# kamenbliznashki/chexpert

Hardware: AMD Instinct MI355X
Metric: images/sec fwd+bwd DenseNet121 320x320 bf16 (per-GPU rate in config.images_per_sec_per_gpu) (higher is better)
Workload: dtype bf16; 1 GPU; densenet121 bf16 1xMI355X 320x320 bs=256 per GPU, U-Ones labels (BASELINE configs[1]); 14 classes; random-init weights, synthetic uint8 X-rays; per_gpu_batch=256, global_batch=256, parallelism=dp1, rccl_ranks=1, capture_failed=0, launch=hipGraph replay

## Files before the change

### chexpert_amd/csrc/conv3x3_strip.hip

```cpp
#include <cstdlib>
#include "common.h"

namespace {

constexpr int XP_FWD = 272;
constexpr int XP_WG = 320;
constexpr int NCHX = 7;

struct StripGeo {
  int B, H, W, P, R, Q;
  int spi;
  int steps_per_wg;
};

__device__ __forceinline__ int wrapq(int v, int q) { return v >= q ? v - q : v; }

__global__ __launch_bounds__(192, 2) void conv3x3_strip_fwd_kernel(const bf16* __restrict__ x, int ldx,
                                                                 const float* __restrict__ sc, const float* __restrict__ sh,
                                                                 const bf16* __restrict__ wpk, bf16* __restrict__ y, int ldy,
                                                                 float* stat_sum, float* stat_sq, int stat_replicas, int stat_rstride,
                                                                 int stat_det, const StripGeo g) {
  extern __shared__ __attribute__((aligned(16))) char smem[];
  float* coef = reinterpret_cast<float*>(smem);
  float* lstat = coef + 256;
  float* scratch = lstat + 64;
  char* ring = reinterpret_cast<char*>(scratch + 3 * 1024);
  const int tid = threadIdx.x, lane = tid & 63, wave = tid >> 6;
  const int P = g.P, R = g.R, Q = g.Q, W = g.W, H = g.H;

  bf16x8 wr[3][8];
#pragma unroll
  for (int dx = 0; dx < 3; ++dx)
#pragma unroll
    for (int ks = 0; ks < 8; ++ks)
      wr[dx][ks] = *reinterpret_cast<const bf16x8*>(wpk + ((size_t)((wave * 3 + dx) * 32 + (lane & 31)) * 128 + ks * 16 + (lane >> 5) * 8));
  for (int i = tid; i < (Q + 2) * (XP_FWD / 16); i += 192) reinterpret_cast<uint4*>(ring)[i] = make_uint4(0, 0, 0, 0);
  for (int i = tid; i < 128; i += 192) { coef[i] = sc[i]; coef[128 + i] = sh[i]; }
  if (tid < 64) lstat[tid] = 0.f;
  __syncthreads();

  const int total_steps = g.B * g.spi;
  const int u0 = blockIdx.x * g.steps_per_wg;
  const int u1 = min(total_steps, u0 + g.steps_per_wg);
  const int chunks_per_row = W * 16;

  uint4 pre[NCHX];
  bool pv[NCHX];
  int base_row = 0;
  int crow[NCHX], cpx[NCHX], cc8[NCHX];
#pragma unroll
  for (int i = 0; i < NCHX; ++i) {
    const int cid = tid + 192 * i;
    crow[i] = cid / chunks_per_row;
    const int rem = cid - crow[i] * chunks_per_row;
    cpx[i] = rem >> 4;
    cc8[i] = rem & 15;
  }
  auto issue_rows = [&](int b, int y0, int n) {
#pragma unroll
    for (int i = 0; i < NCHX; ++i) {
      const int yy = y0 + crow[i];
      pv[i] = crow[i] < n && yy >= 0 && yy < H;
      const int yc_ = min(max(yy, 0), H - 1);
      pre[i] = *reinterpret_cast<const uint4*>(x + ((size_t)(b * H + yc_) * W + cpx[i]) * ldx + cc8[i] * 8);
    }
  };
  auto write_rows = [&](int y0, int n) {
#pragma unroll
    for (int i = 0; i < NCHX; ++i) {
      if (crow[i] < n) {
        int slot = (y0 + crow[i] - base_row) % (R + 2);
        if (slot < 0) slot += R + 2;
        U128 o, v;
        v.u = pre[i];
#pragma unroll
        for (int j = 0; j < 8; ++j)
          o.e[j] = f2bf(fmaxf(fmaf(bf2f(v.e[j]), coef[cc8[i] * 8 + j], coef[128 + cc8[i] * 8 + j]), 0.f));
        { const unsigned keep = pv[i] ? 0xffffffffu : 0u; o.u.x &= keep; o.u.y &= keep; o.u.z &= keep; o.u.w &= keep; }
        const int pos = slot * P + cpx[i] + 1;
        *reinterpret_cast<uint4*>(ring + pos * XP_FWD + cc8[i] * 16) = o.u;
        if (pos < 2) *reinterpret_cast<uint4*>(ring + (Q + pos) * XP_FWD + cc8[i] * 16) = o.u;
      }
    }
  };

  float s1[8], s2[8];
#pragma unroll
  for (int j = 0; j < 8; ++j) s1[j] = s2[j] = 0.f;
  const int nsub = (R * P + 31) / 32;
  bool have_window = false;
  int prev_b = -1, prev_yc = 0;

  for (int u = u0; u < u1; ++u) {
    const int b = u / g.spi, yc = (u - b * g.spi) * R;
    const bool cont = have_window && b == prev_b && yc == prev_yc + R;
    if (!cont) {
      __syncthreads();
      base_row = yc - 1;
      issue_rows(b, yc - 1, 1);
      write_rows(yc - 1, 1);
      issue_rows(b, yc, 1);
      write_rows(yc, 1);
      issue_rows(b, yc + 1, R);
    }
    write_rows(yc + 1, R);
    __syncthreads();
    const bool next_cont = (u + 1 < u1) && ((u + 1) / g.spi == b);
    if (next_cont) issue_rows(b, yc + R + 1, R);
    int slot0 = (yc - 1 - base_row) % (R + 2);
    if (slot0 < 0) slot0 += R + 2;
    const int ws = slot0 * P;

    for (int s = 0; s < nsub; ++s) {
      f32x16 acc;
#pragma unroll
      for (int r = 0; r < 16; ++r) acc[r] = 0.f;
      {
        const int pix = min(s * 32 + (lane & 31), R * P - 1);
        const char* ap = ring + wrapq(wrapq(ws + pix + wave * P, Q), Q) * XP_FWD + (lane >> 5) * 16;
#pragma unroll
        for (int dx = 0; dx < 3; ++dx)
#pragma unroll
          for (int ks = 0; ks < 8; ++ks) {
            const bf16x8 a = *reinterpret_cast<const bf16x8*>(ap + dx * XP_FWD + ks * 32);
            acc = __builtin_amdgcn_mfma_f32_32x32x16_bf16(a, wr[dx][ks], acc, 0, 0, 0);
          }
      }
      float* my = scratch + wave * 1024;
#pragma unroll
      for (int r = 0; r < 16; ++r) my[((r & 3) + 8 * (r >> 2) + 4 * (lane >> 5)) * 32 + (lane & 31)] = acc[r];
      __syncthreads();
      if (tid < 128) {
        const int pr = tid >> 2, c = tid & 3;
        const int m = s * 32 + pr;
        const int oy = m / P, ox = m - oy * P;
        const int yy = yc + oy;
        if (m < R * P && ox < W && yy < H) {
          float v[8];
#pragma unroll
          for (int j = 0; j < 8; ++j) v[j] = 0.f;
#pragma unroll
          for (int w3 = 0; w3 < 3; ++w3) {
            const float4 v0 = *reinterpret_cast<const float4*>(scratch + w3 * 1024 + pr * 32 + c * 8);
            const float4 v1 = *reinterpret_cast<const float4*>(scratch + w3 * 1024 + pr * 32 + c * 8 + 4);
            v[0] += v0.x; v[1] += v0.y; v[2] += v0.z; v[3] += v0.w;
            v[4] += v1.x; v[5] += v1.y; v[6] += v1.z; v[7] += v1.w;
          }
          U128 o;
#pragma unroll
          for (int j = 0; j < 8; ++j) {
            o.e[j] = f2bf(v[j]);
            const float rv = bf2f(o.e[j]);
            s1[j] += rv;
            s2[j] += rv * rv;
          }
          *reinterpret_cast<uint4*>(y + ((size_t)(b * H + yy) * W + ox) * ldy + c * 8) = o.u;
        }
      }
      __syncthreads();
    }
    have_window = true;
    prev_b = b;
    prev_yc = yc;
  }

  if (stat_sum) {
#pragma unroll
    for (int j = 0; j < 8; ++j) {
#pragma unroll
      for (int d = 4; d < 64; d <<= 1) {
        s1[j] += __shfl_xor(s1[j], d);
        s2[j] += __shfl_xor(s2[j], d);
      }
    }
    wg_stat_begin<3>(scratch, 32, tid, 192);
    if (lane < 4 && wave < 2) {
#pragma unroll
      for (int j = 0; j < 8; ++j) wg_stat_put(scratch, 32, wave, lane * 8 + j, s1[j], s2[j]);
    }
    wg_stat_end<3>(scratch, 32, tid, 192, stat_sum, stat_sq, stat_det, (int)blockIdx.x, stat_replicas, stat_rstride, 0, 32);
  }
}

constexpr int GP = 80;
constexpr int NCHD = 2;

__global__ __launch_bounds__(192, 2) void conv3x3_strip_dgrad_kernel(
    const bf16* __restrict__ gsl, int ldg, const bf16* __restrict__ g2, int ldg2, const float* __restrict__ ga,
    const float* __restrict__ gb, const float* __restrict__ gc, const bf16* __restrict__ wpk, const bf16* __restrict__ ex, int ldex,
    const float* __restrict__ e_sc, const float* __restrict__ e_sh, const float* __restrict__ e_mu, const float* __restrict__ e_r,
    const float* __restrict__ e_scale, bf16* __restrict__ y, int ldy, float* S1, float* S2, int stat_replicas, int stat_rstride,
    int stat_det, const StripGeo g) {
  extern __shared__ __attribute__((aligned(16))) char smem[];
  float* coef = reinterpret_cast<float*>(smem);
  float* lstat = coef + 128;
  float* econst = lstat + 256;
  float* scratch = econst + 640;
  char* ring = reinterpret_cast<char*>(scratch + 3 * 4096);
  const int tid = threadIdx.x, lane = tid & 63, wave = tid >> 6;
  const int P = g.P, R = g.R, Q = g.Q, W = g.W, H = g.H;

  bf16x8 wr[3][2][4];
#pragma unroll
  for (int dx = 0; dx < 3; ++dx)
#pragma unroll
    for (int ks = 0; ks < 2; ++ks)
#pragma unroll
      for (int nt = 0; nt < 4; ++nt)
        wr[dx][ks][nt] = *reinterpret_cast<const bf16x8*>(wpk + ((size_t)((wave * 3 + dx) * 128 + nt * 32 + (lane & 31)) * 32 + ks * 16 + (lane >> 5) * 8));
  for (int i = tid; i < (Q + 2) * (GP / 16); i += 192) reinterpret_cast<uint4*>(ring)[i] = make_uint4(0, 0, 0, 0);
  if (tid < 32) { coef[tid] = ga[tid]; coef[32 + tid] = gb[tid]; coef[64 + tid] = gc[tid]; }
  for (int i = tid; i < 256; i += 192) lstat[i] = 0.f;
  const int ec = (tid & 15) * 8;
  float s1[8], s2[8];
#pragma unroll
  for (int j = 0; j < 8; ++j) s1[j] = s2[j] = 0.f;
  if (tid < 128) {
    econst[tid] = e_sc[tid]; econst[128 + tid] = e_sh[tid]; econst[256 + tid] = e_mu[tid]; econst[384 + tid] = e_r[tid];
    econst[512 + tid] = e_scale[tid];
  }
  __syncthreads();

  const int total_steps = g.B * g.spi;
  const int u0 = blockIdx.x * g.steps_per_wg;
  const int u1 = min(total_steps, u0 + g.steps_per_wg);
  const int cpr = W * 4;

  uint4 pg[NCHD], pg2[NCHD];
  bool gv[NCHD];
  int base_row = 0;
  int crow[NCHD], cpx[NCHD], cc8[NCHD];
#pragma unroll
  for (int i = 0; i < NCHD; ++i) {
    const int cid = tid + 192 * i;
    crow[i] = cid / cpr;
    const int rem = cid - crow[i] * cpr;
    cpx[i] = rem >> 2;
    cc8[i] = rem & 3;
  }
  auto issue_rows = [&](int b, int y0, int n) {
#pragma unroll
    for (int i = 0; i < NCHD; ++i) {
      const int yy = y0 + crow[i];
      gv[i] = crow[i] < n && yy >= 0 && yy < H;
      const int yc_ = min(max(yy, 0), H - 1);
      const size_t pixel = (size_t)(b * H + yc_) * W + cpx[i];
      pg[i] = *reinterpret_cast<const uint4*>(gsl + pixel * ldg + cc8[i] * 8);
      pg2[i] = *reinterpret_cast<const uint4*>(g2 + pixel * ldg2 + cc8[i] * 8);
    }
  };
  auto write_rows = [&](int y0, int n) {
#pragma unroll
    for (int i = 0; i < NCHD; ++i) {
      if (crow[i] < n) {
        int slot = (y0 + crow[i] - base_row) % (R + 2);
        if (slot < 0) slot += R + 2;
        U128 o, u, v;
        u.u = pg[i];
        v.u = pg2[i];
#pragma unroll
        for (int j = 0; j < 8; ++j) {
          const float t = fmaf(bf2f(u.e[j]), coef[cc8[i] * 8 + j], fmaf(bf2f(v.e[j]), coef[32 + cc8[i] * 8 + j], coef[64 + cc8[i] * 8 + j]));
          o.e[j] = f2bf(t);
        }
        { const unsigned keep = gv[i] ? 0xffffffffu : 0u; o.u.x &= keep; o.u.y &= keep; o.u.z &= keep; o.u.w &= keep; }
        const int pos = slot * P + cpx[i] + 1;
        *reinterpret_cast<uint4*>(ring + pos * GP + cc8[i] * 16) = o.u;
        if (pos < 2) *reinterpret_cast<uint4*>(ring + (Q + pos) * GP + cc8[i] * 16) = o.u;
      }
    }
  };

  const int nsub = (R * P + 31) / 32;
  bool have_window = false;
  int prev_b = -1, prev_yc = 0;

  for (int u = u0; u < u1; ++u) {
    const int b = u / g.spi, yc = (u - b * g.spi) * R;
    const bool cont = have_window && b == prev_b && yc == prev_yc + R;
    if (!cont) {
      __syncthreads();
      base_row = yc - 1;
      issue_rows(b, yc - 1, 1);
      write_rows(yc - 1, 1);
      issue_rows(b, yc, 1);
      write_rows(yc, 1);
      issue_rows(b, yc + 1, R);
    }
    write_rows(yc + 1, R);
    __syncthreads();
    const bool next_cont = (u + 1 < u1) && ((u + 1) / g.spi == b);
    if (next_cont) issue_rows(b, yc + R + 1, R);
    int slot0 = (yc - 1 - base_row) % (R + 2);
    if (slot0 < 0) slot0 += R + 2;
    const int ws = slot0 * P;

    for (int s = 0; s < nsub; ++s) {
      uint4 exv[3];
      bool exok[3];
      int eoff[3];
#pragma unroll
      for (int i = 0; i < 3; ++i) {
        const int item = tid + 192 * i;
        const int pr = item >> 4;
        const int m = s * 32 + pr;
        const int oy = m / P, ox = m - oy * P;
        const int yy = yc + oy;
        exok[i] = item < 512 && m < R * P && ox < W && yy < H;
        const int oyc = min(yy, H - 1), oxc = min(ox, W - 1);
        eoff[i] = (b * H + oyc) * W + oxc;
        exv[i] = *reinterpret_cast<const uint4*>(ex + (size_t)eoff[i] * ldex + ec);
      }
      f32x16 acc[4];
#pragma unroll
      for (int nt = 0; nt < 4; ++nt)
#pragma unroll
        for (int r = 0; r < 16; ++r) acc[nt][r] = 0.f;
      {
        const int pix = min(s * 32 + (lane & 31), R * P - 1);
        const char* ap = ring + wrapq(wrapq(ws + pix + wave * P, Q), Q) * GP + (lane >> 5) * 16;
#pragma unroll
        for (int dx = 0; dx < 3; ++dx)
#pragma unroll
          for (int ks = 0; ks < 2; ++ks) {
            const bf16x8 a = *reinterpret_cast<const bf16x8*>(ap + dx * GP + ks * 32);
#pragma unroll
            for (int nt = 0; nt < 4; ++nt) acc[nt] = __builtin_amdgcn_mfma_f32_32x32x16_bf16(a, wr[dx][ks][nt], acc[nt], 0, 0, 0);
          }
      }
      float* my = scratch + wave * 4096;
#pragma unroll
      for (int nt = 0; nt < 4; ++nt)
#pragma unroll
        for (int r = 0; r < 16; ++r) my[((r & 3) + 8 * (r >> 2) + 4 * (lane >> 5)) * 128 + nt * 32 + (lane & 31)] = acc[nt][r];
      __syncthreads();
#pragma unroll
      for (int i = 0; i < 3; ++i) {
        const int item = tid + 192 * i;
        const int pr = item >> 4;
        if (exok[i]) {
          float v[8];
#pragma unroll
          for (int j = 0; j < 8; ++j) v[j] = 0.f;
#pragma unroll
          for (int w3 = 0; w3 < 3; ++w3) {
            const float4 v0 = *reinterpret_cast<const float4*>(scratch + w3 * 4096 + pr * 128 + ec);
            const float4 v1 = *reinterpret_cast<const float4*>(scratch + w3 * 4096 + pr * 128 + ec + 4);
            v[0] += v0.x; v[1] += v0.y; v[2] += v0.z; v[3] += v0.w;
            v[4] += v1.x; v[5] += v1.y; v[6] += v1.z; v[7] += v1.w;
          }
          U128 xv, o;
          xv.u = exv[i];
#pragma unroll
          for (int j = 0; j < 8; ++j) {
            const float xf = bf2f(xv.e[j]);
            const float dz = (fmaf(xf, econst[ec + j], econst[128 + ec + j]) > 0.f) ? v[j] : 0.f;
            s1[j] += dz;
            s2[j] += dz * (xf - econst[256 + ec + j]) * econst[384 + ec + j];
            o.e[j] = f2bf(econst[512 + ec + j] * dz);
          }
          *reinterpret_cast<uint4*>(y + (size_t)eoff[i] * ldy + ec) = o.u;
        }
      }
      __syncthreads();
    }
    have_window = true;
    prev_b = b;
    prev_yc = yc;
  }

#pragma unroll
  for (int j = 0; j < 8; ++j) {
    s1[j] += __shfl_xor(s1[j], 16);
    s1[j] += __shfl_xor(s1[j], 32);
    s2[j] += __shfl_xor(s2[j], 16);
    s2[j] += __shfl_xor(s2[j], 32);
  }
  wg_stat_begin<3>(scratch, 128, tid, 192);
  if (lane < 16) {
#pragma unroll
    for (int j = 0; j < 8; ++j) wg_stat_put(scratch, 128, wave, ec + j, s1[j], s2[j]);
  }
  wg_stat_end<3>(scratch, 128, tid, 192, S1, S2, stat_det, (int)blockIdx.x, stat_replicas, stat_rstride, 0, 128);
}

__device__ __forceinline__ bf16x8 tr2(const char* a0, const char* a1) {
  typedef __attribute__((address_space(3))) s16x4 lds_s16x4;
  return cx_join_tr(__builtin_amdgcn_ds_read_tr16_b64_v4i16((lds_s16x4*)(a0)), __builtin_amdgcn_ds_read_tr16_b64_v4i16((lds_s16x4*)(a1)));
}

constexpr int NCHW1 = 5;
constexpr int NCHW4 = 3;
constexpr int WP = 64;

#ifdef CX_STRIP_STAMPS
__device__ unsigned long long strip_stamps[1024 * 8];
__device__ __forceinline__ unsigned long long sstamp() {
  unsigned long long t;
  __builtin_amdgcn_sched_barrier(0);
  asm volatile("s_memtime %0\n\ts_waitcnt lgkmcnt(0)" : "=s"(t)::"memory");
  __builtin_amdgcn_sched_barrier(0);
  return t;
}
#define SSTAMP(i) { const unsigned long long t_ = sstamp(); st_acc[i] += t_ - st_prev; st_prev = t_; }
#else
#define SSTAMP(i)
#endif
template <int NG, int NCHW>
__device__ __forceinline__ void strip_wgrad_body(
    const bf16* __restrict__ gsl, int ldg, const bf16* __restrict__ g2, int ldg2, const float* __restrict__ ga,
    const float* __restrict__ gb, const float* __restrict__ gc, int g_affine2, const bf16* __restrict__ x, int ldx,
    const float* __restrict__ pa, const float* __restrict__ pb, float* __restrict__ dw, const int K, const int N,
    const int c_tiles, const int n_tiles, const StripGeo& g, float* __restrict__ slab, const int wg) {
  extern __shared__ __attribute__((aligned(16))) char smem[];
  const int P = g.P, R = g.R, Q = g.Q, W = g.W, H = g.H;
  const int nk = (R * P + 15) / 16;
  float* coef = reinterpret_cast<float*>(smem);
  char* ring = smem + 160 * 4;
  char* gst = ring + (size_t)(Q + 2) * WP;
  float* red = reinterpret_cast<float*>(ring);
  constexpr int NTHR = 192 * NG;
  const int tid = threadIdx.x, lane = tid & 63;
  const int wave = (tid >> 6) % 3, grp = (tid >> 6) / 3;
  const int pairs = c_tiles * n_tiles;
  const int split = wg / pairs, pair = wg - split * pairs;
  const int nt = pair / c_tiles, ct = pair - nt * c_tiles;
  const int c0 = ct * 32, n0 = nt * 32;
  gsl += n0;
  g2 += n0;

  for (int i = tid; i < ((Q + 2) + nk * 16) * (WP / 16); i += NTHR) reinterpret_cast<uint4*>(ring)[i] = make_uint4(0, 0, 0, 0);
  if (tid < 32) {
    coef[tid] = pa[c0 + tid];
    coef[32 + tid] = pb[c0 + tid];
    const int nn = n0 + tid < N ? n0 + tid : N - 1;
    coef[64 + tid] = g_affine2 ? ga[nn] : 1.f;
    coef[96 + tid] = g_affine2 ? gb[nn] : 0.f;
    coef[128 + tid] = g_affine2 ? gc[nn] : 0.f;
  }
  __syncthreads();

  const int total_steps = g.B * g.spi;
  const int u0 = split * g.steps_per_wg;
  const int u1 = min(total_steps, u0 + g.steps_per_wg);
  const int cpr = W * 4;

  uint4 pre[NCHW], pg[NCHW], pg2[NCHW];
  bool pv[NCHW], gv[NCHW];
  int base_row = 0;
  int crow[NCHW], cpx[NCHW], cc8[NCHW];
#pragma unroll
  for (int i = 0; i < NCHW; ++i) {
    const int cid = tid + NTHR * i;
    crow[i] = cid / cpr;
    const int rem = cid - crow[i] * cpr;
    cpx[i] = rem >> 2;
    cc8[i] = rem & 3;
  }
  uint32_t vox[NCHW], vog[NCHW], vog2[NCHW];
#pragma unroll
  for (int i = 0; i < NCHW; ++i) {
    vox[i] = ((uint32_t)(crow[i] * W + cpx[i]) * (uint32_t)ldx + (uint32_t)(c0 + cc8[i] * 8)) * 2u;
    const int co = n0 + cc8[i] * 8 < N ? cc8[i] * 8 : 0;
    vog[i] = ((uint32_t)(crow[i] * W + cpx[i]) * (uint32_t)ldg + (uint32_t)co) * 2u;
    vog2[i] = ((uint32_t)(crow[i] * W + cpx[i]) * (uint32_t)ldg2 + (uint32_t)co) * 2u;
  }
  const char* __restrict__ xb = reinterpret_cast<const char*>(x);
  const char* __restrict__ gslb = reinterpret_cast<const char*>(gsl);
  const char* __restrict__ g2b = reinterpret_cast<const char*>(g2);
  auto issue_rows_i = [&](int i, uint32_t sx, uint32_t r_lo, uint32_t r_n) __attribute__((always_inline)) {
    pv[i] = ((uint32_t)crow[i] - r_lo) < r_n;
    pre[i] = *reinterpret_cast<const uint4*>(xb + (size_t)(pv[i] ? sx + vox[i] : 0u));
  };
  auto issue_rows = [&](int b, int y0, int n) {
    const uint32_t sx = (uint32_t)((b * H + y0) * W) * (uint32_t)ldx * 2u;
    const uint32_t r_lo = (uint32_t)max(-y0, 0), r_n = (uint32_t)max(min(n, H - y0), 0) - r_lo;
#pragma unroll
    for (int i = 0; i < NCHW; ++i) issue_rows_i(i, sx, r_lo, r_n);
  };
  auto write_rows = [&](int y0, int n) {
#pragma unroll
    for (int i = 0; i < NCHW; ++i) {
      if (crow[i] < n) {
        int slot = (y0 + crow[i] - base_row) % (R + 2);
        if (slot < 0) slot += R + 2;
        U128 o;
        o.u = cx_affine_relu8(pre[i], coef + cc8[i] * 8, coef + 32 + cc8[i] * 8);
        { const unsigned keep = pv[i] ? 0xffffffffu : 0u; o.u.x &= keep; o.u.y &= keep; o.u.z &= keep; o.u.w &= keep; }
        const int pos = slot * P + cpx[i] + 1;
        *reinterpret_cast<uint4*>(ring + pos * WP + cc8[i] * 16) = o.u;
        if (pos < 2) *reinterpret_cast<uint4*>(ring + (Q + pos) * WP + cc8[i] * 16) = o.u;
      }
    }
  };
  auto issue_g_i = [&](int i, uint32_t sg, uint32_t sg2, uint32_t r_n) __attribute__((always_inline)) {
    const bool nok = n0 + cc8[i] * 8 < N;
    gv[i] = (uint32_t)crow[i] < r_n && nok;
    pg[i] = *reinterpret_cast<const uint4*>(gslb + (size_t)(gv[i] ? sg + vog[i] : 0u));
    if (g_affine2) pg2[i] = *reinterpret_cast<const uint4*>(g2b + (size_t)(gv[i] ? sg2 + vog2[i] : 0u));
  };
  auto issue_g = [&](int b, int yc) {
    const uint32_t row0 = (uint32_t)((b * H + yc) * W);
    const uint32_t sg = row0 * (uint32_t)ldg * 2u, sg2 = row0 * (uint32_t)ldg2 * 2u;
    const uint32_t r_n = (uint32_t)max(min(R, H - yc), 0);
#pragma unroll
    for (int i = 0; i < NCHW; ++i) issue_g_i(i, sg, sg2, r_n);
  };
  auto write_g = [&]() {
#pragma unroll
    for (int i = 0; i < NCHW; ++i) {
      if (crow[i] < R) {
        U128 o;
        o.u = g_affine2 ? cx_affine2_8(pg[i], pg2[i], coef + 64 + cc8[i] * 8, coef + 96 + cc8[i] * 8, coef + 128 + cc8[i] * 8) : pg[i];
        { const unsigned keep = gv[i] ? 0xffffffffu : 0u; o.u.x &= keep; o.u.y &= keep; o.u.z &= keep; o.u.w &= keep; }
        *reinterpret_cast<uint4*>(gst + (crow[i] * P + cpx[i]) * WP + cc8[i] * 16) = o.u;
      }
    }
  };

  f32x16 acc[3];
#pragma unroll
  for (int t = 0; t < 3; ++t)
#pragma unroll
    for (int r = 0; r < 16; ++r) acc[t][r] = 0.f;

  const int gq = (lane & 15) >> 2, gp = lane & 3, gg = lane >> 4;
  const int lrow = 8 * (gg >> 1) + gq;
  const int gcol = (16 * (gg & 1) + 4 * gp) * 2;
  const int QB = Q * WP;
  bool have_window = false;
  int prev_b = -1, prev_yc = 0;

#ifdef CX_STRIP_STAMPS
  unsigned long long st_acc[6] = {0, 0, 0, 0, 0, 0}, st_prev = sstamp();
#endif
  for (int u = u0; u < u1; ++u) {
    const int b = u / g.spi, yc = (u - b * g.spi) * R;
    const bool cont = have_window && b == prev_b && yc == prev_yc + R;
    if (!cont) {
      __syncthreads();
      base_row = yc - 1;
      issue_rows(b, yc - 1, 2);
      write_rows(yc - 1, 2);
      issue_rows(b, yc + 1, R);
      issue_g(b, yc);
    }
    SSTAMP(0)
    write_rows(yc + 1, R);
    write_g();
    SSTAMP(1)
    __syncthreads();
    SSTAMP(2)
    const bool next_cont = (u + 1 < u1) && ((u + 1) / g.spi == b);
    SSTAMP(3)
    int slot0 = (yc - 1 - base_row) % (R + 2);
    if (slot0 < 0) slot0 += R + 2;
    const int ws = slot0 * P;
    int o0 = ((ws + lrow + wave * P + grp * 16) % Q) * WP;
    int o1 = ((ws + lrow + 4 + wave * P + grp * 16) % Q) * WP;
    auto kstep = [&](int kk) __attribute__((always_inline)) {
      const char* gbase = gst + (kk * 16 + lrow) * WP + gcol;
      const bf16x8 af = tr2(gbase, gbase + 4 * WP);
#pragma unroll
      for (int dx = 0; dx < 3; ++dx) {
        const bf16x8 bfr = tr2(ring + o0 + gcol + dx * WP, ring + o1 + gcol + dx * WP);
        acc[dx] = __builtin_amdgcn_mfma_f32_32x32x16_bf16(af, bfr, acc[dx], 0, 0, 0);
      }
      o0 += 16 * NG * WP;
      while (o0 >= QB) o0 -= QB;
      o1 += 16 * NG * WP;
      while (o1 >= QB) o1 -= QB;
    };
    int kk = grp;
    if (next_cont) {
      const int yn = yc + R + 1;
      const uint32_t sx = (uint32_t)((b * H + yn) * W) * (uint32_t)ldx * 2u;
      const uint32_t r_lo = (uint32_t)max(-yn, 0), r_nx = (uint32_t)max(min(R, H - yn), 0) - r_lo;
      const uint32_t row0 = (uint32_t)((b * H + yc + R) * W);
      const uint32_t sg = row0 * (uint32_t)ldg * 2u, sg2 = row0 * (uint32_t)ldg2 * 2u;
      const uint32_t r_ng = (uint32_t)max(min(R, H - (yc + R)), 0);
#pragma unroll
      for (int i = 0; i < NCHW; ++i) {
        issue_rows_i(i, sx, r_lo, r_nx);
        issue_g_i(i, sg, sg2, r_ng);
        if (kk < nk) { kstep(kk); kk += NG; }
      }
    }
    for (; kk < nk; kk += NG) kstep(kk);
#ifdef CX_STRIP_STAMPS
    asm volatile("" ::"v"(acc[0][0]), "v"(acc[1][0]), "v"(acc[2][0]));
#endif
    SSTAMP(4)
    __syncthreads();
    SSTAMP(5)
    have_window = true;
    prev_b = b;
    prev_yc = yc;
  }
#ifdef CX_STRIP_STAMPS
  if (tid == 0 && wg < 1024) {
    for (int i = 0; i < 6; ++i) strip_stamps[wg * 8 + i] = st_acc[i];
    strip_stamps[wg * 8 + 6] = (unsigned long long)(u1 - u0);
  }
#endif

  for (int round = 0; round < NG; ++round) {
    if (grp == round) {
#pragma unroll
      for (int dx = 0; dx < 3; ++dx)
#pragma unroll
        for (int r = 0; r < 16; ++r) {
          const int n = (r & 3) + 8 * (r >> 2) + 4 * (lane >> 5);
          float* slot = red + (n * 32 + (lane & 31)) * 9 + wave * 3 + dx;
          *slot = round == 0 ? acc[dx][r] : *slot + acc[dx][r];
        }
    }
    __syncthreads();
  }
  for (int idx = tid; idx < 32 * 288; idx += NTHR) {
    const int n = idx / 288, i = idx - n * 288;
    if (n0 + n < N) dw_out(dw, slab, (size_t)N * K * 9, split, ((size_t)(n0 + n) * K + c0) * 9 + i, red[idx]);
  }
}

template <int NG, int NCHW>
__global__ __launch_bounds__(192 * NG) void conv3x3_strip_wgrad_kernel(
    const bf16* __restrict__ gsl, int ldg, const bf16* __restrict__ g2, int ldg2, const float* __restrict__ ga,
    const float* __restrict__ gb, const float* __restrict__ gc, int g_affine2, const bf16* __restrict__ x, int ldx,
    const float* __restrict__ pa, const float* __restrict__ pb, float* __restrict__ dw, const int K, const int N,
    const int c_tiles, const int n_tiles, const StripGeo g, float* __restrict__ slab) {
  strip_wgrad_body<NG, NCHW>(gsl, ldg, g2, ldg2, ga, gb, gc, g_affine2, x, ldx, pa, pb, dw, K, N, c_tiles, n_tiles, g, slab,
                             xcd_remap(blockIdx.x, gridDim.x));
}

struct StripBatch {
  const bf16* g[CX_WGRAD_BATCH_MAX];
  const bf16* x[CX_WGRAD_BATCH_MAX];
  const float* pa[CX_WGRAD_BATCH_MAX];
  const float* pb[CX_WGRAD_BATCH_MAX];
  float* slab[CX_WGRAD_BATCH_MAX];
};

template <int NG, int NCHW>
__global__ __launch_bounds__(192 * NG) void conv3x3_strip_wgrad_batch_kernel(const StripBatch bt, const int per_layer, int ldg, int ldx,
                                                                             const int K, const int N, const int c_tiles,
                                                                             const int n_tiles, const StripGeo g) {
  const int layer = blockIdx.x / per_layer;
  const int r = blockIdx.x - layer * per_layer;
  const int wg = (per_layer & 7) ? r : xcd_remap(r, per_layer);
  strip_wgrad_body<NG, NCHW>(bt.g[layer], ldg, bt.g[layer], ldg, nullptr, nullptr, nullptr, 0, bt.x[layer], ldx, bt.pa[layer],
                             bt.pb[layer], nullptr, K, N, c_tiles, n_tiles, g, bt.slab[layer], wg);
}

inline StripGeo make_geo(int B, int H, int W, int target_wgs, int min_steps, int max_flat) {
  StripGeo g;
  g.B = B; g.H = H; g.W = W; g.P = W + 2;
  g.R = max_flat / g.P;
  if (g.R < 1) g.R = 1;
  if (g.R > H) g.R = H;
  g.Q = (g.R + 2) * g.P;
  g.spi = (H + g.R - 1) / g.R;
  const int total = B * g.spi;
  int spw = (total + target_wgs - 1) / target_wgs;
  if (spw < min_steps) spw = min_steps;
  if (spw > total) spw = total;
  g.steps_per_wg = spw;
  return g;
}

}

int cx_try_strip_fwd(const CxConv& p, hipStream_t st, bool* handled) {
  *handled = false;
  if (p.mode != CX_MODE_CONV || p.kh != 3 || p.kw != 3 || p.stride != 1 || p.pad != 1) return 0;
  if (p.K != 128 || p.N != 32 || p.prologue != CX_PRO_AFFINE_RELU || p.epilogue != CX_EPI_STORE) return 0;
  if (p.W + 2 > 96 || p.W < 4) return 0;
  StripGeo g = make_geo(p.B, p.H, p.W, 512, 4, 96);
  if (g.R * p.W * 16 > NCHX * 192) return 0;
  const size_t smem = (256 + 64 + 3 * 1024) * 4 + (size_t)(g.Q + 2) * XP_FWD;
  if (smem > 80 * 1024) return 0;
  static bool attr = false;
  if (!attr) {
    (void)hipFuncSetAttribute(reinterpret_cast<const void*>(&conv3x3_strip_fwd_kernel), hipFuncAttributeMaxDynamicSharedMemorySize,
                              80 * 1024);
    attr = true;
  }
  const int total = g.B * g.spi;
  const int grid = (total + g.steps_per_wg - 1) / g.steps_per_wg;
  *handled = true;
  if (const int e = stat_rows_check(p, grid)) return e;
  CX_KTAG("conv3x3_strip_fwd_kernel");
  hipLaunchKernelGGL(conv3x3_strip_fwd_kernel, dim3(grid), dim3(192), smem, st, (const bf16*)p.x, p.ldx, p.pa, p.pb,
                     (const bf16*)p.w, (bf16*)p.y, p.ldy, p.stat_sum, p.stat_sq, p.stat_replicas, p.stat_rstride, p.stat_det, g);
  return launch_status();
}

int cx_try_strip_dgrad(const CxConv& p, hipStream_t st, bool* handled) {
  *handled = false;
  if (p.mode != CX_MODE_CONV || p.kh != 3 || p.kw != 3 || p.stride != 1 || p.pad != 1) return 0;
  if (p.K != 32 || p.N != 128 || p.prologue != CX_PRO_AFFINE2 || p.epilogue != CX_EPI_MASK || p.accumulate) return 0;
  if (p.W + 2 > 96 || p.W < 4) return 0;
  StripGeo g = make_geo(p.B, p.H, p.W, 512, 4, 96);
  if (g.R * p.W * 4 > NCHD * 192) return 0;
  const size_t smem = (128 + 256 + 640 + 3 * 4096) * 4 + (size_t)(g.Q + 2) * GP;
  if (smem > 80 * 1024) return 0;
  static bool attr = false;
  if (!attr) {
    (void)hipFuncSetAttribute(reinterpret_cast<const void*>(&conv3x3_strip_dgrad_kernel), hipFuncAttributeMaxDynamicSharedMemorySize,
                              80 * 1024);
    attr = true;
  }
  const int total = g.B * g.spi;
  const int grid = (total + g.steps_per_wg - 1) / g.steps_per_wg;
  *handled = true;
  if (const int e = stat_rows_check(p, grid)) return e;
  CX_KTAG("conv3x3_strip_dgrad_kernel");
  hipLaunchKernelGGL(conv3x3_strip_dgrad_kernel, dim3(grid), dim3(192), smem, st, (const bf16*)p.x, p.ldx, (const bf16*)p.x2, p.ldx2,
                     p.pa, p.pb, p.pc, (const bf16*)p.w, (const bf16*)p.ex, p.ldex, p.e_sc, p.e_sh, p.e_mu, p.e_r, p.e_scale,
                     (bf16*)p.y, p.ldy, p.stat_sum, p.stat_sq, p.stat_replicas, p.stat_rstride, p.stat_det, g);
  return launch_status();
}

int cx_try_strip_wgrad(const CxWgrad& p, hipStream_t st, bool* handled) {
  *handled = false;
  if (p.mode != CX_MODE_CONV || p.kh != 3 || p.kw != 3 || p.stride != 1 || p.pad != 1) return 0;
  if (p.K % 32 || p.N % 8 || p.K > 2048 || p.N > 2048 || p.x_prologue != CX_PRO_AFFINE_RELU) return 0;
  if (p.g_prologue != CX_PRO_NONE && p.g_prologue != CX_PRO_AFFINE2) return 0;
  if (p.W + 2 > 128 || p.W < 4) return 0;
  {
    unsigned long long ldm = (unsigned long long)(p.ldx > p.ldg ? p.ldx : p.ldg);
    if (p.g_prologue == CX_PRO_AFFINE2 && (unsigned long long)p.ldg2 > ldm) ldm = (unsigned long long)p.ldg2;
    if ((unsigned long long)p.B * p.H * p.W * ldm * 2ull >= (1ull << 32)) return 0;
  }
  const long long px = (long long)p.B * p.H * p.W;
  const int c_tiles = p.K / 32, n_tiles = (p.N + 31) / 32, pairs = c_tiles * n_tiles;
  int wide_splits = 768 / pairs;
  if (wide_splits < 4) wide_splits = 4;
  if (wide_splits > 64) wide_splits = 64;
  const int split_target = pairs == 4 ? 64 : wide_splits;
  {
    int flat = NCHW4 * 768 / (p.W * 4) * (p.W + 2);
    if (flat > 880) flat = 880;
    StripGeo g = make_geo(p.B, p.H, p.W, split_target, 1, flat);
    const int nk = (g.R * g.P + 15) / 16;
    size_t smem = 160 * 4 + (size_t)(g.Q + 2) * WP + (size_t)nk * 16 * WP;
    if (smem < 160 * 4 + 32 * 288 * 4) smem = 160 * 4 + 32 * 288 * 4;
    static const bool off = cx_diag_set("CX_SW_NG1");
    if (!off && g.R * p.W * 4 <= NCHW4 * 768 && 2 * p.W * 4 <= NCHW4 * 768 && g.Q >= 64 && smem <= 150 * 1024) {
      static bool attr = false;
      if (!attr) {
        (void)hipFuncSetAttribute(reinterpret_cast<const void*>(&conv3x3_strip_wgrad_kernel<4, NCHW4>),
                                  hipFuncAttributeMaxDynamicSharedMemorySize, 150 * 1024);
        attr = true;
      }
      const int total = g.B * g.spi;
      const int splits = (total + g.steps_per_wg - 1) / g.steps_per_wg;
      const size_t wtotal = (size_t)p.N * p.K * 9;
      float* slab = dw_slab(p.scratch, p.scratch_floats, splits, (long long)wtotal);
      CX_KTAG("conv3x3_strip_wgrad_kernel<4, %d>", NCHW4);
      hipLaunchKernelGGL((conv3x3_strip_wgrad_kernel<4, NCHW4>), dim3(splits * pairs), dim3(768), smem, st, (const bf16*)p.g, p.ldg,
                         (const bf16*)p.g2, p.ldg2, p.ga, p.gb, p.gc, (int)(p.g_prologue == CX_PRO_AFFINE2), (const bf16*)p.x, p.ldx,
                         p.pa, p.pb, p.dw, p.K, p.N, c_tiles, n_tiles, g, slab);
      *handled = true;
      if (const int e = launch_status()) return e;
      return slab ? cx_dw_reduce(p.dw, slab, wtotal, splits, st) : 0;
    }
  }
  int target = (int)(px / 3200);
  if (target < 64) target = 64;
  if (target > 192) target = 192;
  if (pairs != 4) target = split_target;
  StripGeo g = make_geo(p.B, p.H, p.W, target, 1, 256);
  if (g.R * p.W * 4 > NCHW1 * 192 || 2 * p.W * 4 > NCHW1 * 192 || g.Q < 16) return 0;
  const int nk = (g.R * g.P + 15) / 16;
  size_t smem = 160 * 4 + (size_t)(g.Q + 2) * WP + (size_t)nk * 16 * WP;
  if (smem < 160 * 4 + 32 * 288 * 4) smem = 160 * 4 + 32 * 288 * 4;
  if (smem > 64 * 1024) return 0;
  const int total = g.B * g.spi;
  const int splits = (total + g.steps_per_wg - 1) / g.steps_per_wg;
  const size_t wtotal = (size_t)p.N * p.K * 9;
  float* slab = dw_slab(p.scratch, p.scratch_floats, splits, (long long)wtotal);
  CX_KTAG("conv3x3_strip_wgrad_kernel<1, %d>", NCHW1);
  hipLaunchKernelGGL((conv3x3_strip_wgrad_kernel<1, NCHW1>), dim3(splits * pairs), dim3(192), smem, st, (const bf16*)p.g, p.ldg,
                     (const bf16*)p.g2, p.ldg2, p.ga, p.gb, p.gc, (int)(p.g_prologue == CX_PRO_AFFINE2), (const bf16*)p.x, p.ldx, p.pa, p.pb,
                     p.dw, p.K, p.N, c_tiles, n_tiles, g, slab);
  *handled = true;
  if (const int e = launch_status()) return e;
  return slab ? cx_dw_reduce(p.dw, slab, wtotal, splits, st) : 0;
}

#ifdef CX_STRIP_STAMPS
extern "C" int dbg_strip_stamps(unsigned long long* host, int n_words) {
  return (int)hipMemcpyFromSymbol(host, HIP_SYMBOL(strip_stamps), (size_t)n_words * 8, 0, hipMemcpyDeviceToHost);
}
#endif

int cx_conv3x3_wgrad_batch(const CxWgrad* geo, const CxWgradBatch* items, void* stream) {
  if (!geo || !items) return CX_EINVAL;
  const CxWgrad& p = *geo;
  const int n = items->n;
  if (n <= 0 || n > CX_WGRAD_BATCH_MAX) return CX_EINVAL;
  if (p.dtype != CX_DT_BF16 || p.mode != CX_MODE_CONV || p.kh != 3 || p.kw != 3 || p.stride != 1 || p.pad != 1) return CX_EUNSUPPORTED;
  if (p.K != 128 || p.N != 32 || p.x_prologue != CX_PRO_AFFINE_RELU || p.g_prologue != CX_PRO_NONE) return CX_EUNSUPPORTED;
  if (p.W + 2 > 128 || p.W < 4 || p.Ho != p.H || p.Wo != p.W || (p.ldg % 8) || (p.ldx % 8)) return CX_EUNSUPPORTED;
  if ((unsigned long long)p.B * p.H * p.W * (unsigned long long)(p.ldx > p.ldg ? p.ldx : p.ldg) * 2ull >= (1ull << 32)) return CX_EUNSUPPORTED;
  for (int i = 0; i < n; ++i)
    if (!items->g[i] || !items->x[i] || !items->pa[i] || !items->pb[i] || !items->dw[i]) return CX_EINVAL;
  if (!p.scratch) return CX_EUNSUPPORTED;
  hipStream_t st = as_stream(stream);
  const int c_tiles = 4, n_tiles = 1, pairs = 4;
  static const int env_splits = cx_diag_int("CX_SW_BATCH_SPLITS", 0);
  constexpr int nthr = 768;
  int target = env_splits > 0 ? env_splits : (p.H * p.W > 400 ? 16 : 8);
  int flat = NCHW4 * nthr / (p.W * 4) * (p.W + 2);
  if (flat > 880) flat = 880;
  StripGeo g = make_geo(p.B, p.H, p.W, target, 1, flat);
  const int nk = (g.R * g.P + 15) / 16;
  size_t smem = 160 * 4 + (size_t)(g.Q + 2) * WP + (size_t)nk * 16 * WP;
  if (smem < 160 * 4 + 32 * 288 * 4) smem = 160 * 4 + 32 * 288 * 4;
  if (!(g.R * p.W * 4 <= NCHW4 * nthr && 2 * p.W * 4 <= NCHW4 * nthr && g.Q >= 64 && smem <= 150 * 1024)) return CX_EUNSUPPORTED;
  const int total = g.B * g.spi;
  const int splits = (total + g.steps_per_wg - 1) / g.steps_per_wg;
  const long long wtotal = (long long)p.N * p.K * 9;
  const long long need = (long long)n * splits * wtotal;
  if (need > p.scratch_floats || need >= (1ll << 31)) return CX_EUNSUPPORTED;
  StripBatch bt;
  for (int i = 0; i < CX_WGRAD_BATCH_MAX; ++i) {
    const int j = i < n ? i : 0;
    bt.g[i] = (const bf16*)items->g[j];
    bt.x[i] = (const bf16*)items->x[j];
    bt.pa[i] = items->pa[j];
    bt.pb[i] = items->pb[j];
    bt.slab[i] = p.scratch + (size_t)j * splits * wtotal;
  }
  static bool attr = false;
  if (!attr) {
    (void)hipFuncSetAttribute(reinterpret_cast<const void*>(&conv3x3_strip_wgrad_batch_kernel<4, NCHW4>),
                              hipFuncAttributeMaxDynamicSharedMemorySize, 150 * 1024);
    attr = true;
  }
  const int per_layer = splits * pairs;
  CX_KTAG("conv3x3_strip_wgrad_batch_kernel<4, %d>", NCHW4);
  hipLaunchKernelGGL((conv3x3_strip_wgrad_batch_kernel<4, NCHW4>), dim3(per_layer * n), dim3(768), smem, st, bt, per_layer, p.ldg, p.ldx,
                     p.K, p.N, c_tiles, n_tiles, g);
  if (const int e = launch_status()) return e;
  for (int i = 0; i < n; ++i)
    if (const int e = cx_dw_reduce(items->dw[i], bt.slab[i], (size_t)wtotal, splits, st)) return e;
  cx_tl_slab_floats_v = (int)need;
  return 0;
}
```

### scratch/stamps_strip.py

```python
import ctypes, os, shutil, sys, numpy as np, torch
sys.path.insert(0, '.')
from chexpert_amd import _lib
shutil.copy("scratch/libstamp.so", _lib.LIB_PATH)
from chexpert_amd import ops
dev = torch.device('cuda:0'); bf = torch.bfloat16; B = 256
ops.set_det_wgrad(True)
names = ["restart", "wait+stage", "barrier1", "issue", "multiply", "barrier2"]
for hw, n in ((40, 12), (20, 24), (10, 16)):
    items = []
    for i in range(n):
        g = torch.randn(B, hw, hw, 32, device=dev).to(bf)
        x = torch.randn(B, hw, hw, 128, device=dev).to(bf)
        items.append((g, x, torch.rand(128, device=dev) + 0.5, torch.rand(128, device=dev) - 0.5, torch.zeros(32, 128, 3, 3, device=dev)))
    for _ in range(3):
        ops.wgrad_defer_begin(dev)
        assert ops.conv3x3_wgrad_batch(items)
        ops.wgrad_defer_flush(dev)
    torch.cuda.synchronize()
    host = (ctypes.c_ulonglong * (1024 * 8))()
    ctypes.CDLL(_lib.LIB_PATH).dbg_strip_stamps(host, 1024 * 8)
    a = np.frombuffer(host, dtype=np.uint64).reshape(1024, 8).astype(np.float64)
    a = a[a[:, 6] > 0]
    per = a[:, :6] / a[:, 6:7]
    med = np.median(per, 0)
    print("%dx%d: %d workgroups seen, steps/wg %.0f, core clocks (s_memtime) per step %.1f: " % (hw, hw, len(a), np.median(a[:, 6]), med.sum()) +
          ", ".join("%s %.1f" % (nm, v) for nm, v in zip(names, med)), flush=True)
```

### scratch/trace_step.py

```python
import csv, re, sys
rows = [r for r in csv.DictReader(open(sys.argv[1]))]
rows.sort(key=lambda r: int(r['Start_Timestamp']))
name = lambda r: re.sub(r'\(.*', '', r['Kernel_Name'].replace('void (anonymous namespace)::', '').replace('(anonymous namespace)::', ''))[:48]
idx = [i for i, r in enumerate(rows) if 'adam' in r['Kernel_Name']]
pairs = [(x, y) for x, y in zip(idx, idx[1:]) if y - x > 200]
which = int(sys.argv[2]) if len(sys.argv) > 2 else len(pairs) // 2
a, b = pairs[which]
step = rows[a + 1:b + 1]
t0 = int(step[0]['Start_Timestamp'])
last_end = t0
print("# %d steps; step %d: %d kernels, %.3f ms" % (len(pairs), which, len(step), (int(step[-1]['End_Timestamp']) - t0) / 1e6))
for r in step:
    s, e = int(r['Start_Timestamp']), int(r['End_Timestamp'])
    print("%9.1f %8.1f %7.1f q%-3s %s  g=%s wg=%s" % ((s - t0) / 1e3, (e - s) / 1e3, (s - last_end) / 1e3, r.get('Queue_Id', '?')[-3:], name(r),
                                                   r.get('Grid_Size', r.get('Grid_Size_X', '?')), r.get('Workgroup_Size', r.get('Workgroup_Size_X', '?'))))
    last_end = max(last_end, e)
```

Baseline: 9761 images/sec.

## Prefetch next image's first rows during strip wgrad multiply at image boundaries

After: 9810 images/sec, median of 6. No clear change (+0.5%).

```diff
diff --git a/chexpert_amd/csrc/conv3x3_strip.hip b/chexpert_amd/csrc/conv3x3_strip.hip
--- a/chexpert_amd/csrc/conv3x3_strip.hip
+++ b/chexpert_amd/csrc/conv3x3_strip.hip
@@ -406,7 +406,7 @@
 #else
 #define SSTAMP(i)
 #endif
-template <int NG, int NCHW>
+template <int NG, int NCHW, bool PIPE = false>
 __device__ __forceinline__ void strip_wgrad_body(
     const bf16* __restrict__ gsl, int ldg, const bf16* __restrict__ g2, int ldg2, const float* __restrict__ ga,
     const float* __restrict__ gb, const float* __restrict__ gc, int g_affine2, const bf16* __restrict__ x, int ldx,
@@ -528,7 +528,8 @@
   const int lrow = 8 * (gg >> 1) + gq;
   const int gcol = (16 * (gg & 1) + 4 * gp) * 2;
   const int QB = Q * WP;
-  bool have_window = false;
+  bool have_window = false, fresh = false;
+  uint4 preh = make_uint4(0, 0, 0, 0);
   int prev_b = -1, prev_yc = 0;
 
 #ifdef CX_STRIP_STAMPS
@@ -537,7 +538,7 @@
   for (int u = u0; u < u1; ++u) {
     const int b = u / g.spi, yc = (u - b * g.spi) * R;
     const bool cont = have_window && b == prev_b && yc == prev_yc + R;
-    if (!cont) {
+    if (!cont && !fresh) {
       __syncthreads();
       base_row = yc - 1;
       issue_rows(b, yc - 1, 2);
@@ -546,12 +547,24 @@
       issue_g(b, yc);
     }
     SSTAMP(0)
+    if (fresh) {
+      base_row = -1;
+      if (crow[0] == 0) {
+        U128 o;
+        o.u = cx_affine_relu8(preh, coef + cc8[0] * 8, coef + 32 + cc8[0] * 8);
+        const uint4 z = make_uint4(0, 0, 0, 0);
+        *reinterpret_cast<uint4*>(ring + (cpx[0] + 1) * WP + cc8[0] * 16) = z;
+        if (cpx[0] == 0) *reinterpret_cast<uint4*>(ring + (Q + 1) * WP + cc8[0] * 16) = z;
+        *reinterpret_cast<uint4*>(ring + (P + cpx[0] + 1) * WP + cc8[0] * 16) = o.u;
+      }
+    }
     write_rows(yc + 1, R);
     write_g();
     SSTAMP(1)
     __syncthreads();
     SSTAMP(2)
     const bool next_cont = (u + 1 < u1) && ((u + 1) / g.spi == b);
+    const bool next_fresh = PIPE && u + 1 < u1 && !next_cont;
     SSTAMP(3)
     int slot0 = (yc - 1 - base_row) % (R + 2);
     if (slot0 < 0) slot0 += R + 2;
@@ -572,13 +585,14 @@
       while (o1 >= QB) o1 -= QB;
     };
     int kk = grp;
-    if (next_cont) {
-      const int yn = yc + R + 1;
-      const uint32_t sx = (uint32_t)((b * H + yn) * W) * (uint32_t)ldx * 2u;
+    if (next_cont || next_fresh) {
+      const int bn = next_fresh ? b + 1 : b, yn = next_fresh ? 1 : yc + R + 1, yg = next_fresh ? 0 : yc + R;
+      if (next_fresh) preh = *reinterpret_cast<const uint4*>(xb + (size_t)(crow[0] == 0 ? (uint32_t)(bn * H * W) * (uint32_t)ldx * 2u + vox[0] : 0u));
+      const uint32_t sx = (uint32_t)((bn * H + yn) * W) * (uint32_t)ldx * 2u;
       const uint32_t r_lo = (uint32_t)max(-yn, 0), r_nx = (uint32_t)max(min(R, H - yn), 0) - r_lo;
-      const uint32_t row0 = (uint32_t)((b * H + yc + R) * W);
+      const uint32_t row0 = (uint32_t)((bn * H + yg) * W);
       const uint32_t sg = row0 * (uint32_t)ldg * 2u, sg2 = row0 * (uint32_t)ldg2 * 2u;
-      const uint32_t r_ng = (uint32_t)max(min(R, H - (yc + R)), 0);
+      const uint32_t r_ng = (uint32_t)max(min(R, H - yg), 0);
 #pragma unroll
       for (int i = 0; i < NCHW; ++i) {
         issue_rows_i(i, sx, r_lo, r_nx);
@@ -593,6 +607,7 @@
     SSTAMP(4)
     __syncthreads();
     SSTAMP(5)
+    fresh = next_fresh;
     have_window = true;
     prev_b = b;
     prev_yc = yc;
@@ -648,8 +663,8 @@
   const int layer = blockIdx.x / per_layer;
   const int r = blockIdx.x - layer * per_layer;
   const int wg = (per_layer & 7) ? r : xcd_remap(r, per_layer);
-  strip_wgrad_body<NG, NCHW>(bt.g[layer], ldg, bt.g[layer], ldg, nullptr, nullptr, nullptr, 0, bt.x[layer], ldx, bt.pa[layer],
-                             bt.pb[layer], nullptr, K, N, c_tiles, n_tiles, g, bt.slab[layer], wg);
+  strip_wgrad_body<NG, NCHW, true>(bt.g[layer], ldg, bt.g[layer], ldg, nullptr, nullptr, nullptr, 0, bt.x[layer], ldx, bt.pa[layer],
+                                   bt.pb[layer], nullptr, K, N, c_tiles, n_tiles, g, bt.slab[layer], wg);
 }
 
 inline StripGeo make_geo(int B, int H, int W, int target_wgs, int min_steps, int max_flat) {
diff --git a/scratch/stamps_strip.py b/scratch/stamps_strip.py
--- a/scratch/stamps_strip.py
+++ b/scratch/stamps_strip.py
@@ -6,7 +6,7 @@
 dev = torch.device('cuda:0'); bf = torch.bfloat16; B = 256
 ops.set_det_wgrad(True)
 names = ["restart", "wait+stage", "barrier1", "issue", "multiply", "barrier2"]
-for hw, n in ((40, 12), (20, 24), (10, 16)):
+for hw, n in ((10, 16), (20, 24), (40, 12)):
     items = []
     for i in range(n):
         g = torch.randn(B, hw, hw, 32, device=dev).to(bf)
diff --git a/scratch/trace_step.py b/scratch/trace_step.py
--- a/scratch/trace_step.py
+++ b/scratch/trace_step.py
@@ -2,7 +2,7 @@
 rows = [r for r in csv.DictReader(open(sys.argv[1]))]
 rows.sort(key=lambda r: int(r['Start_Timestamp']))
 name = lambda r: re.sub(r'\(.*', '', r['Kernel_Name'].replace('void (anonymous namespace)::', '').replace('(anonymous namespace)::', ''))[:48]
-idx = [i for i, r in enumerate(rows) if 'adam' in r['Kernel_Name']]
+idx = [i for i, r in enumerate(rows) if 'adam' in r['Kernel_Name'] or '::step_kernel' in r['Kernel_Name']]
 pairs = [(x, y) for x, y in zip(idx, idx[1:]) if y - x > 200]
 which = int(sys.argv[2]) if len(sys.argv) > 2 else len(pairs) // 2
 a, b = pairs[which]
```
